# dobraczka/kiez

Hardware: AMD Instinct MI355X
Metric: source queries/sec (fit+kneighbors) + recall@k vs reference, 1/2/4/8 GPU (higher is better)
Workload: dtype f16

## Files before the change

kiez_amd/csrc/kz_knn_finalize.h:

```cpp
#pragma once


struct KnnFinParams {
    const float* in_key;
    const int* in_idx;
    KzListLayout lay;
    int max_m;
    int fast_div;
    int64_t q_first, q_last;
    int KP;
    int KSEL;
    int64_t list_row0;
    int64_t q_begin;
    int64_t q_count;
    const void* qraw;
    const void* yraw;
    const double* ynorm64;
    const double* qsqn;
    const double* ysqn;
    int64_t n_i;
    int d;
    int metric;
    int k;
    int exclude_self;
    const int64_t* self_ids;
    double gamma;
    const double* ystats;
    int tier_h;
    double eps_mult;
    double gamma_acc;
    const double* q_rowq;
    const double* y_hmax;
    const double* hscale;
    const float* excl_floor;
    const float* list_floor;
    int dual_col;
    const int* idx_map;
    const int* row_map;
    double* out_dist;
    int64_t* out_ind;
    int* fail_count;
    int* fail_list;
    double* fail_tau;
    unsigned long long* err_ratio_bits;
};

template <typename T>
__device__ __forceinline__ double kz_output_distance(double v, int metric, double p = 2.0) {
    if (metric == KZ_MINKOWSKI) return kz_f32_rows<T> ? (double)(float)pow(v, 1.0 / p) : pow(v, 1.0 / p);
    if (metric == KZ_SEUCLIDEAN) return kz_f32_rows<T> ? (double)(float)sqrt(v) : sqrt(v);
    if ((metric == KZ_CORRELATION || metric == KZ_DICE || metric == KZ_SOKALSNEATH) && v == INFINITY) return NAN;
    if (metric == KZ_EUCLIDEAN) {
        if (kz_f32_rows<T>) return (double)(float)sqrt((double)(float)v);
        return sqrt(v);
    }
    return v;
}

template <typename T>
__device__ __forceinline__ void kz_emit_sorted(const double* sval, const int* sidx, int n_sorted, int k, int exclude_self,
                                               int64_t self_row, int metric, double* od, int64_t* oi, int lane, double p = 2.0) {
    int self_rank = -1;
    if (exclude_self) {
        self_rank = 0;
        const int lim = min(n_sorted, k + 1);
        for (int c = 0; c < lim; ++c)
            if ((int64_t)sidx[c] == self_row) {
                self_rank = c;
                break;
            }
    }
    for (int c = lane; c < n_sorted; c += 64) {
        if (c == self_rank) continue;
        const int o = (self_rank >= 0 && c > self_rank) ? c - 1 : c;
        if (o < k) {
            od[o] = kz_output_distance<T>(sval[c], metric, p);
            oi[o] = (int64_t)sidx[c];
        }
    }
}

#ifndef KZ_FIN_ROWS_N
#define KZ_FIN_ROWS_N 1
#endif
#ifndef KZ_FIN_DEPTH
#define KZ_FIN_DEPTH 3
#endif
constexpr int KZ_FIN_ROWS = KZ_FIN_ROWS_N;
__host__ __device__ __forceinline__ int kz_fin_wide_wave_bytes(int max_m, int KS) {
    return ((max_m * 8 + KS * 20) + 15) & ~15;
}

template <int E>
__device__ __forceinline__ float kz_full_lists_bound(const float (&key)[E], const bool (&ok)[E], int M, int KP, int lane) {
    float bound = -INFINITY;
#pragma unroll
    for (int i = 0; i < E; ++i) {
        if (64 * i >= M) break;
        int c = ok[i] ? 1 : 0;
        float mn = ok[i] ? key[i] : INFINITY;
        for (int off = KP >> 1; off >= 1; off >>= 1) {
            c += __shfl_xor(c, off, 64);
            mn = fminf(mn, __shfl_xor(mn, off, 64));
        }
        if (c == KP && lane + 64 * i < M) bound = fmaxf(bound, mn);
    }
#pragma unroll
    for (int off = 32; off >= 1; off >>= 1) bound = fmaxf(bound, __shfl_xor(bound, off, 64));
    return bound;
}

template <int E>
__device__ __forceinline__ unsigned kz_radix_kth_u32_regs(const unsigned (&x)[E], unsigned all_or, unsigned all_and, int rank) {
#pragma unroll
    for (int off = 32; off >= 1; off >>= 1) {
        all_or |= __shfl_xor(all_or, off, 64);
        all_and &= __shfl_xor(all_and, off, 64);
    }
    const unsigned differ = all_or ^ all_and;
    const int top = differ ? 31 - __clz(differ) : -1;
    unsigned thr = top >= 31 ? 0u : (top < 0 ? all_and : (all_and & ~((2u << top) - 1u)));
    for (int bit = top; bit >= 0; --bit) {
        const unsigned cand = thr | (1u << bit);
        int c = 0;
#pragma unroll
        for (int i = 0; i < E; ++i) c += (int)__popcll(__ballot(x[i] >= cand));
        if (c >= rank) thr = cand;
    }
    return thr;
}
template <int E>
__device__ __forceinline__ unsigned kz_radix_kth_u32_e(const unsigned* u, int n, int rank, int lane) {
    unsigned x[E];
    unsigned all_or = 0u, all_and = 0xffffffffu;
#pragma unroll
    for (int i = 0; i < E; ++i) {
        const int e = lane + 64 * i;
        const bool in = e < n;
        x[i] = in ? u[e] : 0u;
        all_or |= x[i];
        all_and &= in ? x[i] : 0xffffffffu;
    }
    return kz_radix_kth_u32_regs<E>(x, all_or, all_and, rank);
}
template <bool REGS = false>
__device__ __forceinline__ unsigned kz_radix_kth_u32(const unsigned* u, int n, int rank, int lane) {
    if (REGS && n <= 256) return kz_radix_kth_u32_e<4>(u, n, rank, lane);
    if (REGS && n <= 512) return kz_radix_kth_u32_e<8>(u, n, rank, lane);
    unsigned all_or = 0u, all_and = 0xffffffffu;
    for (int e = lane; e < n; e += 64) {
        all_or |= u[e];
        all_and &= u[e];
    }
#pragma unroll
    for (int off = 32; off >= 1; off >>= 1) {
        all_or |= __shfl_xor(all_or, off, 64);
        all_and &= __shfl_xor(all_and, off, 64);
    }
    const unsigned differ = all_or ^ all_and;
    const int top = differ ? 31 - __clz(differ) : -1;
    unsigned thr = top >= 31 ? 0u : (top < 0 ? all_and : (all_and & ~((2u << top) - 1u)));
    for (int bit = top; bit >= 0; --bit) {
        const unsigned cand = thr | (1u << bit);
        int c = 0;
        for (int e0 = 0; e0 < n; e0 += 64) c += (int)__popcll(__ballot(e0 + lane < n && u[e0 + lane] >= cand));
        if (c >= rank) thr = cand;
    }
    return thr;
}
template <int E>
__device__ __forceinline__ unsigned long long kz_radix_kth_small_f64_e(const double* v, int n, int rank, int lane) {
    unsigned long long x[E];
    unsigned long long all_or = 0ull, all_and = ~0ull;
#pragma unroll
    for (int i = 0; i < E; ++i) {
        const int e = lane + 64 * i;
        const bool in = e < n;
        x[i] = in ? (unsigned long long)__double_as_longlong(v[e]) : ~0ull;
        all_or |= in ? x[i] : 0ull;
        all_and &= x[i];
    }
#pragma unroll
    for (int off = 32; off >= 1; off >>= 1) {
        all_or |= __shfl_xor(all_or, off, 64);
        all_and &= __shfl_xor(all_and, off, 64);
    }
    const unsigned long long differ = all_or ^ all_and;
    const int top = differ ? 63 - __clzll(differ) : -1;
    unsigned long long thr = top >= 63 ? 0ull : (top < 0 ? all_and : (all_and & ~((2ull << top) - 1ull)));
    for (int bit = top; bit >= 0; --bit) {
        const unsigned long long cand = thr | (1ull << bit);
        int c = 0;
#pragma unroll
        for (int i = 0; i < E; ++i) c += (int)__popcll(__ballot(x[i] < cand));
        if (c < rank) thr = cand;
    }
    return thr;
}
template <bool REGS = false>
__device__ __forceinline__ unsigned long long kz_radix_kth_small_f64(const double* v, int n, int rank, int lane) {
    if (REGS && n <= 256) return kz_radix_kth_small_f64_e<4>(v, n, rank, lane);
    unsigned long long all_or = 0ull, all_and = ~0ull;
    for (int e = lane; e < n; e += 64) {
        const unsigned long long b = (unsigned long long)__double_as_longlong(v[e]);
        all_or |= b;
        all_and &= b;
    }
#pragma unroll
    for (int off = 32; off >= 1; off >>= 1) {
        all_or |= __shfl_xor(all_or, off, 64);
        all_and &= __shfl_xor(all_and, off, 64);
    }
    const unsigned long long differ = all_or ^ all_and;
    const int top = differ ? 63 - __clzll(differ) : -1;
    unsigned long long thr = top >= 63 ? 0ull : (top < 0 ? all_and : (all_and & ~((2ull << top) - 1ull)));
    for (int bit = top; bit >= 0; --bit) {
        const unsigned long long cand = thr | (1ull << bit);
        int c = 0;
        for (int e0 = 0; e0 < n; e0 += 64)
            c += (int)__popcll(__ballot(e0 + lane < n && (unsigned long long)__double_as_longlong(v[e0 + lane]) < cand));
        if (c < rank) thr = cand;
    }
    return thr;
}

template <int E>
__device__ __forceinline__ int kz_rank_select(const float* ekey, const int* eidx, int M, int KP, float* ck, int* ci, int lane) {
    float x[E];
    int xi[E], rank[E];
#pragma unroll
    for (int u = 0; u < E; ++u) {
        const int e = lane + 64 * u;
        x[u] = e < M ? ekey[e] : -INFINITY;
        xi[u] = e < M ? eidx[e] : -1;
        rank[u] = 0;
    }
    int n_valid = 0;
#pragma unroll
    for (int v = 0; v < E; ++v) {
        n_valid += __popcll(__ballot(xi[v] >= 0));
        const int lim = min(64, M - 64 * v);
        for (int jj = 0; jj < lim; ++jj) {
            const int oi = __builtin_amdgcn_readlane(xi[v], jj);
            if (oi < 0) continue;
            const float ox = __uint_as_float((unsigned)__builtin_amdgcn_readlane((int)__float_as_uint(x[v]), jj));
#pragma unroll
            for (int u = 0; u < E; ++u)
                if (64 * u < M) rank[u] += (ox > x[u] || (ox == x[u] && oi < xi[u])) ? 1 : 0;
        }
    }
#pragma unroll
    for (int u = 0; u < E; ++u) {
        if (xi[u] >= 0 && rank[u] < KP) {
            ck[rank[u]] = x[u];
            ci[rank[u]] = xi[u];
        }
    }
    return n_valid < KP ? n_valid : KP;
}

template <typename T, int FROWS, int NV = 1>
__device__ __forceinline__ void kz_finalize_query(const KnnFinParams& p, const int64_t q, const int lane, char* wbase) {
    const int KS = p.KSEL > 0 ? p.KSEL : p.KP;
    double* cv = reinterpret_cast<double*>(wbase);
    double* sv = cv + KS;
    float* ekey = reinterpret_cast<float*>(sv + KS);
    int* eidx = reinterpret_cast<int*>(ekey + p.max_m);
    float* ck = reinterpret_cast<float*>(eidx + p.max_m);
    int* ci = reinterpret_cast<int*>(ck + KS);
    int* si = ci + KS;
    const int KP = p.KP;
    const int k_eff = p.k + (p.exclude_self ? 1 : 0);
    const int64_t qrow = p.row_map ? (int64_t)p.row_map[p.q_begin + q] : p.q_begin + q;
    const int64_t qout = p.row_map ? qrow : q;
    const T* qptr = reinterpret_cast<const T*>(p.qraw) + qrow * (int64_t)p.d;
    const double qs = p.qsqn[qrow];

    const int64_t lrow = p.list_row0 + q;
    const int n_pieces = p.lay.pieces[kz_list_region(lrow, p.lay)];
    const int halves = p.lay.halves;
    const int M = n_pieces * halves * KP;
    if (p.lay.contig) {
        const int64_t l0 = kz_list_contig_off(lrow, p.lay, KP, 0);
        for (int e = lane; e < M; e += 64) {
            ekey[e] = p.in_key[l0 + e];
            int r = p.in_idx[l0 + e];
            if (p.idx_map && r >= 0) r = p.idx_map[r];
            eidx[e] = r;
        }
    } else {
        const int64_t lwave = kz_list_wave_base(lrow, p.lay, KP, 0) + (lrow & 31);
        for (int e = lane; e < M; e += 64) {
            const int piece = e / (halves * KP);
            const int rem = e - piece * halves * KP;
            const int hh = rem / KP;
            const int ee = rem - hh * KP;
            const int64_t off = lwave + ((int64_t)piece * KP + ee) * KZ_LSTRIDE + hh * 32;
            ekey[e] = p.in_key[off];
            eidx[e] = p.in_idx[off];
        }
    }
    kz_wave_sync();

    float piece_bound = p.list_floor ? p.list_floor[p.q_begin + q] : -INFINITY;
    if (KS > KP) {
        for (int l0 = 0; l0 < M; l0 += KP) {
            float mn = INFINITY;
            int cnt = 0;
            for (int e = lane; e < KP; e += 64) {
                const bool ok = eidx[l0 + e] >= 0;
                cnt += ok ? 1 : 0;
                mn = ok ? fminf(mn, ekey[l0 + e]) : mn;
            }
#pragma unroll
            for (int off = 32; off >= 1; off >>= 1) {
                cnt += __shfl_xor(cnt, off, 64);
                mn = fminf(mn, __shfl_xor(mn, off, 64));
            }
            if (cnt == KP) piece_bound = fmaxf(piece_bound, mn);
        }
    }
    int V = 0;
    bool unsorted = false;
    float sel_min = INFINITY, left_max = -INFINITY;
    if (M <= 64) {
        V = kz_rank_select<1>(ekey, eidx, M, KS, ck, ci, lane);
    } else {
        unsorted = true;
        unsigned* uk = reinterpret_cast<unsigned*>(ekey);
        auto key_of = [](unsigned u) { return __uint_as_float(u ^ ((u >> 31) ? 0x80000000u : 0xffffffffu)); };
        int nv = 0;
        for (int e = lane; e < M; e += 64) {
            unsigned bts = __float_as_uint(ekey[e]);
            if (bts == 0x80000000u) bts = 0u;
            const bool valid = eidx[e] >= 0;
            uk[e] = valid ? (bts ^ ((bts >> 31) ? 0xffffffffu : 0x80000000u)) : 0u;
            nv += valid ? 1 : 0;
        }
#pragma unroll
        for (int off = 32; off >= 1; off >>= 1) nv += __shfl_xor(nv, off, 64);
        kz_wave_sync();
        const bool all = nv <= KS;
        unsigned thr = 0u;
        if (!all) thr = kz_radix_kth_u32(uk, M, KS, lane);
        for (int e0 = 0; e0 < M; e0 += 64) {
            const int e = e0 + lane;
            const bool sel = e < M && eidx[e] >= 0 && (all || uk[e] > thr);
            const unsigned long long mask = __ballot(sel);
            if (sel) {
                const int pos = V + (int)__builtin_amdgcn_mbcnt_hi((unsigned)(mask >> 32), __builtin_amdgcn_mbcnt_lo((unsigned)mask, 0u));
                const float kf = key_of(uk[e]);
                ck[pos] = kf;
                ci[pos] = eidx[e];
                sel_min = fminf(sel_min, kf);
            }
            V += (int)__popcll(mask);
        }
        if (!all) {
            int last = -1;
            while (V < KS) {
                int best = 0x7fffffff;
                for (int e = lane; e < M; e += 64) {
                    const int xi = eidx[e];
                    if (xi >= 0 && uk[e] == thr && xi > last && xi < best) best = xi;
                }
#pragma unroll
                for (int off = 32; off >= 1; off >>= 1) best = min(best, __shfl_xor(best, off, 64));
                if (best == 0x7fffffff) break;
                if (lane == 0) {
                    ck[V] = key_of(thr);
                    ci[V] = best;
                }
                last = best;
                ++V;
                sel_min = fminf(sel_min, key_of(thr));
            }
        }
#pragma unroll
        for (int off = 32; off >= 1; off >>= 1) sel_min = fminf(sel_min, __shfl_xor(sel_min, off, 64));
    }
    kz_wave_sync();

    double eps_q, key_scale = 1.0, qref = qs;
    const bool cosine_plain = p.metric == KZ_COSINE && !p.tier_h;
    if (p.tier_h) {
        const double qc2 = p.q_rowq[qrow * 3 + 0], qh = p.q_rowq[qrow * 3 + 1], qr = p.q_rowq[qrow * 3 + 2];
        const double Yh = p.y_hmax[0], Ry = p.y_hmax[1], Yc2 = p.y_hmax[2];
        const double qc = sqrt(qc2), yc = sqrt(Yc2);
        const double ymax = p.ystats[0];
        const double raw2 = p.metric == KZ_COSINE ? 2.0 : qs + ymax * ymax;
        eps_q = p.eps_mult * (qr * Yh + qh * Ry + qr * Ry + p.gamma_acc * (0.5 * Yc2 + qh * Yh) +
                              1.1920928955078125e-07 * (qc + yc) * (qc + yc) + 1e-12 * (0.5 * Yc2 + qc2) + 1e-14 * raw2);
        if (p.dual_col) eps_q += p.eps_mult * (p.gamma_acc * 0.5 * qc2 + 1.1920928955078125e-07 * (0.5 * Yc2 + 0.5 * qc2 + qh * Yh));
        key_scale = p.hscale[1];
        qref = qc2;
    } else if (p.metric == KZ_COSINE) {
        eps_q = p.gamma * 1.001;
    } else {
        const double ymax = p.ystats[0];
        const double scale = 0.5 * ymax * ymax + sqrt(qs) * ymax;
        eps_q = p.gamma * scale;
        if (scale < 1e-30) eps_q = INFINITY;
    }
    auto exact_key = [&](double v) {
        if (cosine_plain) return 1.0 - v;
        return 0.5 * (qref - (p.metric == KZ_COSINE ? 2.0 * v : v));
    };

    int Vr = V;
    if (unsorted) {
        if (V > k_eff && eps_q < INFINITY) {
            unsigned* su = reinterpret_cast<unsigned*>(sv);
            for (int c = lane; c < V; c += 64) {
                unsigned b = __float_as_uint(ck[c]);
                if (b == 0x80000000u) b = 0u;
                su[c] = b ^ ((b >> 31) ? 0xffffffffu : 0x80000000u);
            }
            kz_wave_sync();
            const unsigned uk_k = kz_radix_kth_u32(su, V, k_eff, lane);
            const float key_k = __uint_as_float(uk_k ^ ((uk_k >> 31) ? 0x80000000u : 0xffffffffu));
            const double thr = (double)key_k * key_scale - 2.0 * eps_q;
            int cnt = 0;
            for (int c0 = 0; c0 < V; c0 += 64) {
                const int c = c0 + lane;
                const bool in = c < V && (double)ck[c] * key_scale >= thr;
                const unsigned long long mask = __ballot(in);
                if (in) {
                    const int pos = cnt + (int)__builtin_amdgcn_mbcnt_hi((unsigned)(mask >> 32), __builtin_amdgcn_mbcnt_lo((unsigned)mask, 0u));
                    ekey[pos] = ck[c];
                    eidx[pos] = ci[c];
                } else if (c < V) {
                    left_max = fmaxf(left_max, ck[c]);
                }
                cnt += (int)__popcll(mask);
            }
#pragma unroll
            for (int off = 32; off >= 1; off >>= 1) left_max = fmaxf(left_max, __shfl_xor(left_max, off, 64));
            Vr = cnt;
            ck = ekey;
            ci = eidx;
            kz_wave_sync();
        }
    } else if (V > k_eff && eps_q < INFINITY) {
        const double thr = (double)ck[k_eff - 1] * key_scale - 2.0 * eps_q;
        int cnt = 0;
        for (int c = lane; c < V; c += 64) cnt += ((double)ck[c] * key_scale >= thr) ? 1 : 0;
#pragma unroll
        for (int off = 32; off >= 1; off >>= 1) cnt += __shfl_xor(cnt, off, 64);
        Vr = cnt < k_eff ? k_eff : cnt;
    }

    const T* yraw = reinterpret_cast<const T*>(p.yraw);
    const bool vec = kz_row_vec_ok(qptr, p.d) && kz_row_vec_ok(yraw, p.d);
#ifdef KZ_NO_FIN_PIPE
    if (false) {
#else
    if ((kz_f32_rows<T> || kz_half_rows<T>) && vec && p.d <= 256 * NV && Vr > 0) {
#endif
        const int k0 = 4 * lane;
        bool act[NV];
        int k0r[NV];
        double qk[4 * NV];
#pragma unroll
        for (int c = 0; c < NV; ++c) {
            act[c] = k0 + 256 * c < p.d;
            k0r[c] = act[c] ? k0 + 256 * c : 0;
            double t[4] = {0.0, 0.0, 0.0, 0.0};
            if (act[c]) {
                kz_row4(qptr, k0r[c], p.d, true, t);
                if (p.metric == KZ_COSINE) {
#pragma unroll
                    for (int e = 0; e < 4; ++e) t[e] = t[e] / qs;
                }
            }
#pragma unroll
            for (int e = 0; e < 4; ++e) qk[4 * c + e] = t[e];
        }
        using Frag = KzRowFrag<T>;
        auto issue = [&](int c0, Frag (&buf)[FROWS][NV], double (&ysb)[FROWS]) {
#pragma unroll
            for (int u = 0; u < FROWS; ++u) {
                const int yi = ci[min(c0 + u, Vr - 1)];
                ysb[u] = p.ysqn[yi];
#pragma unroll
                for (int c = 0; c < NV; ++c)
                    buf[u][c] = *reinterpret_cast<const Frag*>(yraw + (int64_t)yi * p.d + k0r[c]);
            }
        };
        auto reduce = [&](int c0, const Frag (&buf)[FROWS][NV], const double (&ysb)[FROWS]) {
#pragma unroll
            for (int u = 0; u < FROWS; ++u) {
                double a = 0.0;
                bool done = false;
                if (p.metric == KZ_COSINE && p.fast_div) {
                    const double rcp = 1.0 / ysb[u];
                    const int rcp_hi = __builtin_amdgcn_readfirstlane((int)((unsigned long long)__double_as_longlong(rcp) >> 32));
                    if ((rcp_hi & 0x7ff00000) != 0x7ff00000) {
#pragma unroll
                        for (int c = 0; c < NV; ++c) {
                            double yk[4];
                            kz_frag4<T>(buf[u][c], yk);
                            if (act[c]) {
#pragma unroll
                                for (int e = 0; e < 4; ++e) a = fma(qk[4 * c + e], kz_div_shared(yk[e], ysb[u], rcp), a);
                            }
                        }
                        done = true;
                    }
                }
                if (!done) {
#pragma unroll
                    for (int c = 0; c < NV; ++c) {
                        double yk[4];
                        kz_frag4<T>(buf[u][c], yk);
                        if (act[c]) {
                            if (p.metric == KZ_COSINE) {
#pragma unroll
                                for (int e = 0; e < 4; ++e) a = fma(qk[4 * c + e], yk[e] / ysb[u], a);
                            } else {
#pragma unroll
                                for (int e = 0; e < 4; ++e) a = fma(qk[4 * c + e], yk[e], a);
                            }
                        }
                    }
                }
                const double dot = kz_wave_sum(a);
                double v;
                if (p.metric == KZ_COSINE) {
                    v = fmin(fmax(1.0 - dot, 0.0), 2.0);
                } else {
                    v = fmax((qs + ysb[u]) - 2.0 * dot, 0.0);
                }
                if (lane == 0 && c0 + u < Vr) cv[c0 + u] = v;
            }
        };
#if KZ_FIN_DEPTH == 3
        constexpr int R = FROWS;
        Frag b0[R][NV], b1[R][NV], b2[R][NV];
        double y0[R], y1[R], y2[R];
        issue(0, b0, y0);
        issue(R, b1, y1);
        for (int c0 = 0;;) {
            issue(c0 + 2 * R, b2, y2);
            reduce(c0, b0, y0);
            if ((c0 += R) >= Vr) break;
            issue(c0 + 2 * R, b0, y0);
            reduce(c0, b1, y1);
            if ((c0 += R) >= Vr) break;
            issue(c0 + 2 * R, b1, y1);
            reduce(c0, b2, y2);
            if ((c0 += R) >= Vr) break;
        }
#else
        Frag cur[FROWS][NV], nxt[FROWS][NV];
        double ys_c[FROWS], ys_n[FROWS];
        issue(0, cur, ys_c);
        for (int c0 = 0; c0 < Vr; c0 += 2 * FROWS) {
            issue(c0 + FROWS, nxt, ys_n);
            reduce(c0, cur, ys_c);
            if (c0 + FROWS >= Vr) break;
            issue(c0 + 2 * FROWS, cur, ys_c);
            reduce(c0 + FROWS, nxt, ys_n);
        }
#endif
    } else
    for (int c0 = 0; c0 < Vr; c0 += FROWS) {
        const T* yp[FROWS];
        double ys[FROWS], acc[FROWS];
#pragma unroll
        for (int u = 0; u < FROWS; ++u) {
            const int yi = ci[min(c0 + u, Vr - 1)];
            yp[u] = yraw + (int64_t)yi * p.d;
            ys[u] = p.ysqn[yi];
            acc[u] = 0.0;
        }
        for (int k0 = 4 * lane; k0 < p.d; k0 += 256) {
            double qk[4];
            kz_row4(qptr, k0, p.d, vec, qk);
            if (p.metric == KZ_COSINE) {
#pragma unroll
                for (int e = 0; e < 4; ++e) qk[e] = qk[e] / qs;
            }
#pragma unroll
            for (int u = 0; u < FROWS; ++u) {
                double yk[4];
                kz_row4(yp[u], k0, p.d, vec, yk);
                if (p.metric == KZ_COSINE) {
#pragma unroll
                    for (int e = 0; e < 4; ++e) acc[u] = fma(qk[e], yk[e] / ys[u], acc[u]);
                } else {
#pragma unroll
                    for (int e = 0; e < 4; ++e) acc[u] = fma(qk[e], yk[e], acc[u]);
                }
            }
        }
#pragma unroll
        for (int u = 0; u < FROWS; ++u) {
            const double dot = kz_wave_sum(acc[u]);
            double v;
            if (p.metric == KZ_COSINE) {
                v = fmin(fmax(1.0 - dot, 0.0), 2.0);
            } else {
                v = fmax((qs + ys[u]) - 2.0 * dot, 0.0);
            }
            if (lane == 0 && c0 + u < Vr) cv[c0 + u] = v;
        }
    }
    kz_wave_sync();
    for (int c = lane; c < Vr; c += 64) {
        const double v = cv[c];
        const int id = ci[c];
        int rank = 0;
        for (int o = 0; o < Vr; ++o) {
            const double ov = cv[o];
            const int oid = ci[o];
            rank += (ov < v || (ov == v && oid < id)) ? 1 : 0;
        }
        sv[rank] = v;
        si[rank] = id;
    }
    kz_wave_sync();

    bool bound_violated = false;
    if (eps_q > 0.0 && eps_q < INFINITY && p.err_ratio_bits) {
        double worst = 0.0;
        for (int c = lane; c < Vr; c += 64) {
            const double v = cv[c];
            if (v > 0.0)
                worst = fmax(worst, fabs((double)ck[c] * key_scale - exact_key(v)) / eps_q);
        }
#pragma unroll
        for (int off = 32; off >= 1; off >>= 1) worst = fmax(worst, __shfl_xor(worst, off, 64));
        bound_violated = worst > 1.0;
        if (lane == 0 && worst > 0.0) {
            const unsigned long long bits = (unsigned long long)__double_as_longlong(worst);
            if (bits > *(const volatile unsigned long long*)p.err_ratio_bits) atomicMax(p.err_ratio_bits, bits);
        }
    }

    bool certified;
    if (p.excl_floor) {
        double bound = (double)p.excl_floor[qrow];
        if (V == KP) bound = fmax(bound, (double)(unsorted ? sel_min : ck[KP - 1]));
        certified = V >= k_eff && bound * key_scale + eps_q < exact_key(sv[k_eff - 1]);
    } else {
        float bound = piece_bound;
        if (V == KS) bound = fmaxf(bound, unsorted ? sel_min : ck[KS - 1]);
        if (bound == -INFINITY)
            certified = (V >= min((int64_t)k_eff, p.n_i));
        else
            certified = V >= k_eff && (double)bound * key_scale + eps_q < exact_key(sv[k_eff - 1]);
    }
    if (Vr < V && !((double)(unsorted ? left_max : ck[Vr]) * key_scale + eps_q < exact_key(sv[k_eff - 1]))) certified = false;
    if (bound_violated) certified = false;
    if (!certified) {
        if (lane == 0) {
            const int pos = atomicAdd(p.fail_count, 1);
            p.fail_list[pos] = (int)qout;
            if (p.fail_tau) p.fail_tau[pos] = Vr >= k_eff ? sv[k_eff - 1] : (double)INFINITY;
        }
        return;
    }
    kz_emit_sorted<T>(sv, si, Vr, p.k, p.exclude_self, p.self_ids ? p.self_ids[q] : qrow, p.metric,
                      p.out_dist + qout * (int64_t)p.k, p.out_ind + qout * (int64_t)p.k, lane);
}

constexpr int KZ_FIN_QPB = 4;
#ifndef KZ_FIN_WAVES_2
#define KZ_FIN_WAVES_2 5
#endif
#ifndef KZ_FIN_WAVES
#define KZ_FIN_WAVES 7
#endif
template <typename T, int FROWS, int MINW, int NV = 1>
__global__ __launch_bounds__(256, MINW) void kz_knn_finalize_kernel(KnnFinParams p) {
    extern __shared__ __attribute__((aligned(16))) char fsm[];
    const int lane = threadIdx.x & 63;
    const int wave = __builtin_amdgcn_readfirstlane(threadIdx.x >> 6);
    char* wbase = fsm + (size_t)wave * kz_fin_wave_bytes(p.max_m, p.KSEL > 0 ? p.KSEL : p.KP);
    for (int rep = 0; rep < KZ_FIN_QPB / 4; ++rep) {
        const int64_t q = p.q_first + (int64_t)blockIdx.x * KZ_FIN_QPB + rep * 4 + wave;
        if (q >= p.q_last) break;
        kz_finalize_query<T, FROWS, NV>(p, q, lane, wbase);
        kz_wave_sync();
    }
}

#include "kz_knn_fin_wide.h"

static int kz_launch_finalize(kz_ctx* ctx, KnnFinParams& fp, const KzListLayout& lay, int KP, int64_t q_count, int dtype) {
    struct Group { int64_t lo, hi; int max_m; } groups[KZ_MAX_REGIONS];
    int n_groups = 0;
    for (int rg = 0; rg < lay.n_regions; ++rg) {
        const int64_t lo = (int64_t)(rg > 0 ? lay.qt_end[rg - 1] : 0) * KZ_TILE - fp.list_row0;
        while (rg + 1 < lay.n_regions && lay.pieces[rg + 1] == lay.pieces[rg]) ++rg;
        const int64_t hi = (int64_t)lay.qt_end[rg] * KZ_TILE - fp.list_row0;
        Group g = {lo < 0 ? 0 : lo, hi > q_count ? q_count : hi, lay.pieces[rg] * lay.halves * KP};
        if (g.hi > g.lo) groups[n_groups++] = g;
    }
    const hipStream_t main_stream = ctx->stream;
    const bool fork = n_groups >= 2 && ctx->stream2 && ctx->stream2 != main_stream && !ctx->stream2_busy;
    int big = 0;
    for (int g = 1; g < n_groups; ++g)
        if (groups[g].hi - groups[g].lo > groups[big].hi - groups[big].lo) big = g;
    const bool wide = (fp.KSEL > 0 ? fp.KSEL : KP) > 160;
    const bool rows_vec = fp.d <= 256 && (fp.d & 3) == 0 && (((uintptr_t)fp.qraw | (uintptr_t)fp.yraw) & 15u) == 0;
    const bool wide2 = wide && dtype == KZ_F32 && fp.tier_h && !fp.excl_floor && rows_vec;
    const bool two_chunks = !wide && (dtype == KZ_F32 || kz_dtype_is_half(dtype)) && fp.d > 256 && fp.d <= 512 && (fp.d & 3) == 0 &&
                            (((uintptr_t)fp.qraw | (uintptr_t)fp.yraw) & (dtype == KZ_F32 ? 15u : 7u)) == 0;
    const void* fk = nullptr;
    if (dtype != KZ_F32) {
        const int rcd = kz_dispatch_rows(dtype, "kz_knn", [&](auto e) {
            using T = typename decltype(e)::type;
            if constexpr (kz_half_rows<T>) {
                if (two_chunks) {
                    fk = (const void*)kz_knn_finalize_kernel<T, KZ_FIN_ROWS, KZ_FIN_WAVES_2, 2>;
                    return (int)KZ_OK;
                }
            }
            fk = wide ? (const void*)kz_knn_finalize_kernel<T, 4, 2> : (const void*)kz_knn_finalize_kernel<T, KZ_FIN_ROWS, KZ_FIN_WAVES>;
            return (int)KZ_OK;
        });
        if (rcd != KZ_OK) return rcd;
    } else if (wide2)
        fk = (const void*)kz_knn_finalize_wide_kernel<float, 4>;
    else if (wide)
        fk = (const void*)kz_knn_finalize_kernel<float, 8, 2>;
    else if (two_chunks)
        fk = (const void*)kz_knn_finalize_kernel<float, KZ_FIN_ROWS, KZ_FIN_WAVES_2, 2>;
    else
        fk = (const void*)kz_knn_finalize_kernel<float, KZ_FIN_ROWS, KZ_FIN_WAVES>;
    if (fork) {
        KZ_HIP(hipEventRecord(ctx->ev[7], main_stream));
        KZ_HIP(hipStreamWaitEvent(ctx->stream2, ctx->ev[7], 0));
    }
    for (int pass = 0; pass < 2; ++pass) {
        for (int g = 0; g < n_groups; ++g) {
            const bool side = fork && g != big;
            if (fork ? (side != (pass == 0)) : pass == 1) continue;
            const hipStream_t st = side ? ctx->stream2 : main_stream;
            fp.q_first = groups[g].lo;
            fp.q_last = groups[g].hi;
            fp.max_m = groups[g].max_m;
            fp.fast_div = ctx->fin_fast_div;
            const int fin_blocks = (int)((fp.q_last - fp.q_first + KZ_FIN_QPB - 1) / KZ_FIN_QPB);
            size_t fin_lds = (size_t)4 * kz_fin_wave_bytes(fp.max_m, fp.KSEL > 0 ? fp.KSEL : KP);
            if (wide2) fin_lds = (size_t)4 * kz_fin_wide_wave_bytes(fp.max_m, fp.KSEL);
            if (fin_lds > 65536) KZ_HIP(hipFuncSetAttribute(fk, hipFuncAttributeMaxDynamicSharedMemorySize, (int)fin_lds));
            void* args[] = {&fp};
            KZ_HIP(hipLaunchKernel(fk, dim3(fin_blocks), dim3(256), args, fin_lds, st));
        }
    }
    KZ_HIP(hipGetLastError());
    if (fork) {
        KZ_HIP(hipEventRecord(ctx->ev[11], ctx->stream2));
        KZ_HIP(hipStreamWaitEvent(main_stream, ctx->ev[11], 0));
    }
    return KZ_OK;
}
```

Measured before the change: 2.913 million.

## Batch wave reductions across row groups using DPP and permlane swaps in rerank

Replaces the per-candidate full 64-lane wave sum in the finalize rerank with a grouped butterfly reduction. Four candidate rows share the exchange levels, so each lane ends up holding one row's dot product, and DPP and permlane swap instructions stand in for generic shuffles. It also specializes the rerank loop on the metric and fast-div mode at compile time, and makes the candidate index and norm loads wave-uniform (readfirstlane plus a constant-address-space load) so they can use scalar loads. The cost is more complex indexing, padding of the final group, and a changed floating-point summation order.

Result: no change. 2.933 million, median of 6 (+0.7%).

```diff
diff --git a/kiez_amd/csrc/kz_knn_finalize.h b/kiez_amd/csrc/kz_knn_finalize.h
--- a/kiez_amd/csrc/kz_knn_finalize.h
+++ b/kiez_amd/csrc/kz_knn_finalize.h
@@ -1,4 +1,5 @@
 #pragma once
+#include "kz_wave_reduce.h"
 
 
 struct KnnFinParams {
@@ -87,6 +88,9 @@
 #define KZ_FIN_DEPTH 3
 #endif
 constexpr int KZ_FIN_ROWS = KZ_FIN_ROWS_N;
+#ifndef KZ_FIN_GROUP
+#define KZ_FIN_GROUP 4
+#endif
 __host__ __device__ __forceinline__ int kz_fin_wide_wave_bytes(int max_m, int KS) {
     return ((max_m * 8 + KS * 20) + 15) & ~15;
 }
@@ -450,6 +454,7 @@
         Vr = cnt < k_eff ? k_eff : cnt;
     }
 
+    Vr = __builtin_amdgcn_readfirstlane(Vr);
     const T* yraw = reinterpret_cast<const T*>(p.yraw);
     const bool vec = kz_row_vec_ok(qptr, p.d) && kz_row_vec_ok(yraw, p.d);
 #ifdef KZ_NO_FIN_PIPE
@@ -480,89 +485,112 @@
         auto issue = [&](int c0, Frag (&buf)[FROWS][NV], double (&ysb)[FROWS]) {
 #pragma unroll
             for (int u = 0; u < FROWS; ++u) {
-                const int yi = ci[min(c0 + u, Vr - 1)];
-                ysb[u] = p.ysqn[yi];
+                const int yi = __builtin_amdgcn_readfirstlane(ci[min(c0 + u, Vr - 1)]);
+                ysb[u] = *(const __attribute__((address_space(4))) double*)(p.ysqn + yi);
 #pragma unroll
                 for (int c = 0; c < NV; ++c)
                     buf[u][c] = *reinterpret_cast<const Frag*>(yraw + (int64_t)yi * p.d + k0r[c]);
             }
         };
-        auto reduce = [&](int c0, const Frag (&buf)[FROWS][NV], const double (&ysb)[FROWS]) {
-#pragma unroll
-            for (int u = 0; u < FROWS; ++u) {
-                double a = 0.0;
-                bool done = false;
-                if (p.metric == KZ_COSINE && p.fast_div) {
-                    const double rcp = 1.0 / ysb[u];
-                    const int rcp_hi = __builtin_amdgcn_readfirstlane((int)((unsigned long long)__double_as_longlong(rcp) >> 32));
-                    if ((rcp_hi & 0x7ff00000) != 0x7ff00000) {
+        KzWaveGroupSum<KZ_FIN_GROUP> grp;
+        const int my_row = kz_wr_lane_row(KZ_FIN_GROUP, lane);
+        const bool writes = kz_wr_lane_writes(KZ_FIN_GROUP, lane);
+        double ys_mine = 0.0;
+        auto rerank = [&](auto mode_tag) {
+            constexpr int MODE = decltype(mode_tag)::value;
+            auto close = [&](int c_last) {
+                const double dot = grp.total;
+                double v;
+                if constexpr (MODE != 0) {
+                    v = fmin(fmax(1.0 - dot, 0.0), 2.0);
+                } else {
+                    v = fmax((qs + ys_mine) - 2.0 * dot, 0.0);
+                }
+                const int c = c_last - (KZ_FIN_GROUP - 1) + my_row;
+                if (writes && c < Vr) cv[c] = v;
+            };
+            auto reduce = [&](int c0, const Frag (&buf)[FROWS][NV], const double (&ysb)[FROWS]) {
+#pragma unroll
+                for (int u = 0; u < FROWS; ++u) {
+                    double a = 0.0;
+                    bool done = false;
+                    if constexpr (MODE == 1) {
+                        const double rcp = 1.0 / ysb[u];
+                        const int rcp_hi = __builtin_amdgcn_readfirstlane((int)((unsigned long long)__double_as_longlong(rcp) >> 32));
+                        if ((rcp_hi & 0x7ff00000) != 0x7ff00000) {
+#pragma unroll
+                            for (int c = 0; c < NV; ++c) {
+                                double yk[4];
+                                kz_frag4<T>(buf[u][c], yk);
+                                if (act[c]) {
+#pragma unroll
+                                    for (int e = 0; e < 4; ++e) a = fma(qk[4 * c + e], kz_div_shared(yk[e], ysb[u], rcp), a);
+                                }
+                            }
+                            done = true;
+                        }
+                    }
+                    if (!done) {
 #pragma unroll
                         for (int c = 0; c < NV; ++c) {
                             double yk[4];
                             kz_frag4<T>(buf[u][c], yk);
                             if (act[c]) {
-#pragma unroll
-                                for (int e = 0; e < 4; ++e) a = fma(qk[4 * c + e], kz_div_shared(yk[e], ysb[u], rcp), a);
-                            }
-                        }
-                        done = true;
-                    }
-                }
-                if (!done) {
-#pragma unroll
-                    for (int c = 0; c < NV; ++c) {
-                        double yk[4];
-                        kz_frag4<T>(buf[u][c], yk);
-                        if (act[c]) {
-                            if (p.metric == KZ_COSINE) {
-#pragma unroll
-                                for (int e = 0; e < 4; ++e) a = fma(qk[4 * c + e], yk[e] / ysb[u], a);
-                            } else {
-#pragma unroll
-                                for (int e = 0; e < 4; ++e) a = fma(qk[4 * c + e], yk[e], a);
+                                if constexpr (MODE != 0) {
+#pragma unroll
+                                    for (int e = 0; e < 4; ++e) a = fma(qk[4 * c + e], yk[e] / ysb[u], a);
+                                } else {
+#pragma unroll
+                                    for (int e = 0; e < 4; ++e) a = fma(qk[4 * c + e], yk[e], a);
+                                }
                             }
                         }
                     }
+                    if constexpr (MODE == 0) ys_mine = ((c0 + u) & (KZ_FIN_GROUP - 1)) == my_row ? ysb[u] : ys_mine;
+                    if (grp.feed(a, lane)) close(c0 + u);
                 }
-                const double dot = kz_wave_sum(a);
-                double v;
-                if (p.metric == KZ_COSINE) {
-                    v = fmin(fmax(1.0 - dot, 0.0), 2.0);
-                } else {
-                    v = fmax((qs + ysb[u]) - 2.0 * dot, 0.0);
-                }
-                if (lane == 0 && c0 + u < Vr) cv[c0 + u] = v;
-            }
+            };
+#if KZ_FIN_DEPTH == 3
+            constexpr int R = FROWS;
+            Frag b0[R][NV], b1[R][NV], b2[R][NV];
+            double y0[R], y1[R], y2[R];
+            issue(0, b0, y0);
+            issue(R, b1, y1);
+            int c0 = 0;
+            for (;;) {
+                issue(c0 + 2 * R, b2, y2);
+                reduce(c0, b0, y0);
+                if ((c0 += R) >= Vr) break;
+                issue(c0 + 2 * R, b0, y0);
+                reduce(c0, b1, y1);
+                if ((c0 += R) >= Vr) break;
+                issue(c0 + 2 * R, b1, y1);
+                reduce(c0, b2, y2);
+                if ((c0 += R) >= Vr) break;
+            }
+#else
+            Frag cur[FROWS][NV], nxt[FROWS][NV];
+            double ys_c[FROWS], ys_n[FROWS];
+            issue(0, cur, ys_c);
+            int c0 = 0;
+            for (;;) {
+                issue(c0 + FROWS, nxt, ys_n);
+                reduce(c0, cur, ys_c);
+                if ((c0 += FROWS) >= Vr) break;
+                issue(c0 + FROWS, cur, ys_c);
+                reduce(c0, nxt, ys_n);
+                if ((c0 += FROWS) >= Vr) break;
+            }
+#endif
+            for (; c0 & (KZ_FIN_GROUP - 1); ++c0)
+                if (grp.feed(0.0, lane)) close(c0);
         };
-#if KZ_FIN_DEPTH == 3
-        constexpr int R = FROWS;
-        Frag b0[R][NV], b1[R][NV], b2[R][NV];
-        double y0[R], y1[R], y2[R];
-        issue(0, b0, y0);
-        issue(R, b1, y1);
-        for (int c0 = 0;;) {
-            issue(c0 + 2 * R, b2, y2);
-            reduce(c0, b0, y0);
-            if ((c0 += R) >= Vr) break;
-            issue(c0 + 2 * R, b0, y0);
-            reduce(c0, b1, y1);
-            if ((c0 += R) >= Vr) break;
-            issue(c0 + 2 * R, b1, y1);
-            reduce(c0, b2, y2);
-            if ((c0 += R) >= Vr) break;
-        }
-#else
-        Frag cur[FROWS][NV], nxt[FROWS][NV];
-        double ys_c[FROWS], ys_n[FROWS];
-        issue(0, cur, ys_c);
-        for (int c0 = 0; c0 < Vr; c0 += 2 * FROWS) {
-            issue(c0 + FROWS, nxt, ys_n);
-            reduce(c0, cur, ys_c);
-            if (c0 + FROWS >= Vr) break;
-            issue(c0 + 2 * FROWS, cur, ys_c);
-            reduce(c0 + FROWS, nxt, ys_n);
-        }
-#endif
+        if (p.metric != KZ_COSINE)
+            rerank(std::integral_constant<int, 0>());
+        else if (p.fast_div)
+            rerank(std::integral_constant<int, 1>());
+        else
+            rerank(std::integral_constant<int, 2>());
     } else
     for (int c0 = 0; c0 < Vr; c0 += FROWS) {
         const T* yp[FROWS];
diff --git a/kiez_amd/csrc/kz_wave_reduce.h b/kiez_amd/csrc/kz_wave_reduce.h
--- /dev/null
+++ b/kiez_amd/csrc/kz_wave_reduce.h
@@ -0,0 +1,158 @@
+#pragma once
+
+#if defined(__HIPCC__)
+#define KZ_WR_FN __host__ __device__ constexpr
+#else
+#define KZ_WR_FN constexpr
+#endif
+
+KZ_WR_FN int kz_wr_levels(int G) { return G <= 1 ? 0 : 1 + kz_wr_levels(G >> 1); }
+KZ_WR_FN int kz_wr_offset(int level) { return 32 >> level; }
+KZ_WR_FN bool kz_wr_keeps_first(int level, int lane) { return ((lane >> (5 - level)) & 1) == 0; }
+KZ_WR_FN int kz_wr_lane_row(int G, int lane) {
+    int row = 0;
+    for (int j = 0; j < kz_wr_levels(G); ++j) row |= ((lane >> (5 - j)) & 1) << j;
+    return row;
+}
+KZ_WR_FN bool kz_wr_lane_writes(int G, int lane) { return (lane & (64 / G - 1)) == 0; }
+KZ_WR_FN int kz_wr_writer_lane(int G, int row) {
+    int lane = 0;
+    for (int j = 0; j < kz_wr_levels(G); ++j) lane |= ((row >> j) & 1) << (5 - j);
+    return lane;
+}
+KZ_WR_FN int kz_wr_merges(int G, int u) {
+    int n = 0;
+    while (n < kz_wr_levels(G) && ((u >> n) & 1)) ++n;
+    return n;
+}
+
+template <int G>
+struct KzWaveGroupModel {
+    static constexpr int L = kz_wr_levels(G);
+    double wait[L > 0 ? L : 1][64];
+    double total[64];
+    int n = 0;
+
+    static void merge(int level, const double* first, const double* second, double* out) {
+        const int off = kz_wr_offset(level);
+        double r[64];
+        for (int l = 0; l < 64; ++l) {
+            const int p = l ^ off;
+            if (off >= 16)
+                r[l] = kz_wr_keeps_first(level, l) ? first[l] + first[p] : second[p] + second[l];
+            else
+                r[l] = kz_wr_keeps_first(level, l) ? first[l] + first[p] : second[l] + second[p];
+        }
+        for (int l = 0; l < 64; ++l) out[l] = r[l];
+    }
+    bool feed(const double* a) {
+        double t[64];
+        for (int l = 0; l < 64; ++l) t[l] = a[l];
+        const int m = kz_wr_merges(G, n);
+        for (int j = 0; j < m; ++j) merge(j, wait[j], t, t);
+        if (n != G - 1) {
+            for (int l = 0; l < 64; ++l) wait[m][l] = t[l];
+            ++n;
+            return false;
+        }
+        for (int j = L; j < 6; ++j) {
+            if (kz_wr_offset(j) >= 16) {
+                merge(j, t, t, t);
+                continue;
+            }
+            double r[64];
+            for (int l = 0; l < 64; ++l) r[l] = t[l] + t[l ^ kz_wr_offset(j)];
+            for (int l = 0; l < 64; ++l) t[l] = r[l];
+        }
+        for (int l = 0; l < 64; ++l) total[l] = t[l];
+        n = 0;
+        return true;
+    }
+};
+
+#if defined(__HIPCC__)
+__device__ __forceinline__ void kz_wr_split(double x, int& lo, int& hi) {
+    const long long b = __double_as_longlong(x);
+    lo = (int)b;
+    hi = (int)(b >> 32);
+}
+__device__ __forceinline__ double kz_wr_join(int lo, int hi) {
+    return __longlong_as_double((long long)(((unsigned long long)(unsigned)hi << 32) | (unsigned)lo));
+}
+template <int OFF>
+__device__ __forceinline__ int kz_wr_xor_lane_b32(int x) {
+    static_assert(OFF == 8 || OFF == 4 || OFF == 2 || OFF == 1, "DPP exchanges stay inside a row of 16 lanes");
+    if constexpr (OFF == 8) return __builtin_amdgcn_mov_dpp(x, 0x128, 0xf, 0xf, true);
+    if constexpr (OFF == 4) return __builtin_amdgcn_mov_dpp(__builtin_amdgcn_mov_dpp(x, 0x141, 0xf, 0xf, true), 0x1b, 0xf, 0xf, true);
+    if constexpr (OFF == 2) return __builtin_amdgcn_mov_dpp(x, 0x4e, 0xf, 0xf, true);
+    return __builtin_amdgcn_mov_dpp(x, 0xb1, 0xf, 0xf, true);
+}
+template <int OFF>
+__device__ __forceinline__ double kz_wr_xor_lane(double x) {
+    int lo, hi;
+    kz_wr_split(x, lo, hi);
+    return kz_wr_join(kz_wr_xor_lane_b32<OFF>(lo), kz_wr_xor_lane_b32<OFF>(hi));
+}
+template <int LEVEL>
+__device__ __forceinline__ double kz_wr_merge(double first, double second, int lane) {
+    constexpr int OFF = kz_wr_offset(LEVEL);
+    if constexpr (OFF >= 16) {
+        int flo, fhi, slo, shi;
+        kz_wr_split(first, flo, fhi);
+        kz_wr_split(second, slo, shi);
+        if constexpr (OFF == 32) {
+            const auto a = __builtin_amdgcn_permlane32_swap((unsigned)flo, (unsigned)slo, false, false);
+            const auto b = __builtin_amdgcn_permlane32_swap((unsigned)fhi, (unsigned)shi, false, false);
+            return kz_wr_join((int)a[0], (int)b[0]) + kz_wr_join((int)a[1], (int)b[1]);
+        } else {
+            const auto a = __builtin_amdgcn_permlane16_swap((unsigned)flo, (unsigned)slo, false, false);
+            const auto b = __builtin_amdgcn_permlane16_swap((unsigned)fhi, (unsigned)shi, false, false);
+            return kz_wr_join((int)a[0], (int)b[0]) + kz_wr_join((int)a[1], (int)b[1]);
+        }
+    } else {
+        const bool kf = kz_wr_keeps_first(LEVEL, lane);
+        const double keep = kf ? first : second, send = kf ? second : first;
+        return keep + kz_wr_xor_lane<OFF>(send);
+    }
+}
+
+template <int G>
+struct KzWaveGroupSum {
+    static_assert(G == 1 || G == 2 || G == 4 || G == 8 || G == 16, "groups of 1 to 16 rows");
+    static constexpr int L = kz_wr_levels(G);
+    double wait[L > 0 ? L : 1];
+    double total;
+    int n = 0;
+
+    template <int J>
+    __device__ __forceinline__ void step(double t, int lane) {
+        if constexpr (J < L) {
+            if ((n >> J) & 1) {
+                step<J + 1>(kz_wr_merge<J>(wait[J], t, lane), lane);
+            } else {
+                wait[J] = t;
+            }
+        } else {
+            finish<L>(t, lane);
+        }
+    }
+    template <int J>
+    __device__ __forceinline__ void finish(double t, int lane) {
+        if constexpr (J < 6) {
+            if constexpr (kz_wr_offset(J) >= 16) {
+                finish<J + 1>(kz_wr_merge<J>(t, t, lane), lane);
+            } else {
+                finish<J + 1>(t + kz_wr_xor_lane<kz_wr_offset(J)>(t), lane);
+            }
+        } else {
+            total = t;
+        }
+    }
+    __device__ __forceinline__ bool feed(double a, int lane) {
+        step<0>(a, lane);
+        const bool complete = (n & (G - 1)) == G - 1;
+        ++n;
+        return complete;
+    }
+};
+#endif
```
